# distributed-lab/era-boojum

Hardware: AMD Instinct MI355X
Metric: LDE+Merkle commit Goldilocks elems/s (2^22x256, LDE x4) (higher is better)
Workload: dtype u64 (Goldilocks); 1 GPU; C3: 2^22 rows x 256 cols, LDE x4, Poseidon2 cap 16; rows=4194304, cols=256, lde=4, cap=16, tree_hasher=poseidon2, parallelism=single, launch=stream

## Files before the change

### era-boojum_amd/csrc/bj_internal.hpp

```cpp
#pragma once
#include <hip/hip_runtime.h>
#include <stdint.h>
#include <stddef.h>
#include <stdlib.h>
#include <string.h>

namespace bj {

struct Knobs {
    bool enabled;
    uint64_t leaves_defer;
    uint64_t leaves_group;
    uint64_t inv_fold_unpaired;
    uint64_t lde_passes;
    uint64_t node_q4_max;
    uint64_t node_fused;
    uint64_t lde_own_fused;
};
inline Knobs read_knobs() {
    Knobs k{false, 0, 0, 0, 3, (uint64_t)1 << 15, 1, 1};
    const char* g = getenv("BJ_EXPERIMENTS");
    k.enabled = g && strcmp(g, "1") == 0;
    if (!k.enabled) return k;
    const char* e;
    if ((e = getenv("BJ_LEAVES_DEFER"))) k.leaves_defer = strtoull(e, nullptr, 0);
    if ((e = getenv("BJ_LEAVES_GROUP"))) k.leaves_group = strtoull(e, nullptr, 0);
    if ((e = getenv("BJ_INV_FOLD_UNPAIRED"))) k.inv_fold_unpaired = e[0] == '1';
    if ((e = getenv("BJ_LDE_PASSES"))) k.lde_passes = e[0] == '2' ? 2 : 3;
    if ((e = getenv("BJ_NODE_Q4_MAX"))) k.node_q4_max = strtoull(e, nullptr, 0);
    if ((e = getenv("BJ_NODE_FUSED"))) k.node_fused = e[0] != '0';
    if ((e = getenv("BJ_LDE_OWN_FUSED"))) k.lde_own_fused = e[0] != '0';
    return k;
}
inline const Knobs& knobs() {
    static const Knobs k = read_knobs();
    return k;
}

hipError_t launch_bitrev_scale(uint64_t* dst, size_t dst_stride, const uint64_t* src, size_t src_stride,
                               uint32_t n_cols, uint32_t log_n, uint64_t scale, hipStream_t st);
hipError_t launch_twiddles(uint64_t* out, uint32_t log_n, bool inverse, hipStream_t st);
hipError_t launch_twiddles_natural(uint64_t* out, uint32_t log_n, bool inverse, hipStream_t st);
hipError_t launch_bitrev_inplace(uint64_t* cols, size_t col_stride, uint32_t n_cols, uint32_t log_n, hipStream_t st);
hipError_t launch_power_tables(uint64_t* lo, uint64_t* hi, uint32_t log_n, uint64_t e, uint64_t scale,
                               hipStream_t st);
hipError_t launch_distribute(uint64_t* cols, size_t col_stride, uint32_t n_cols, uint32_t log_n,
                             const uint64_t* lo, const uint64_t* hi, hipStream_t st);

hipError_t launch_leaves(const uint64_t* src, size_t col_stride, uint32_t n_cols, size_t n_leaves, uint64_t* out,
                         hipStream_t st);
hipError_t launch_leaves_partial(const uint64_t* src, size_t col_stride, uint32_t n_cols, size_t n_leaves,
                                 const uint64_t* cap_in, uint64_t* out, bool final_, hipStream_t st);
hipError_t launch_leaves_chunked(const uint64_t* src, size_t col_stride, uint32_t n_cols, uint32_t log_e,
                                 size_t n_leaves, uint64_t* out, hipStream_t st);
hipError_t launch_nodes(const uint64_t* leaves, size_t n_leaves, uint32_t cap_size, uint64_t* nodes,
                        hipStream_t st);
hipError_t launch_permute(uint64_t* states, size_t count, hipStream_t st);
hipError_t launch_synthetic(uint64_t* dst, size_t col_stride, uint32_t n_cols, uint32_t log_n, uint64_t seed,
                            uint64_t col0, hipStream_t st);

hipError_t launch_gl_op(int op, const uint64_t* a, const uint64_t* b, uint64_t* out, size_t n, hipStream_t st);

hipError_t launch_twiddle_pyramid(uint64_t* out, uint32_t log_n, bool inverse, hipStream_t st);
hipError_t launch_dif(uint64_t* dst, size_t dst_stride, const uint64_t* src, size_t src_stride, uint32_t n_cols,
                      uint32_t log_n, const uint64_t* tw_pyr, bool canon_out, hipStream_t st);
hipError_t launch_lde_forward(uint64_t* lde, size_t lde_col_stride, uint32_t n_cosets, const uint64_t* raw,
                              size_t raw_stride, bool raw_bitrev, uint32_t n_cols, uint32_t log_n,
                              const uint64_t* tw_pyr, const uint64_t* pw, size_t pw_stride, hipStream_t st);

inline size_t pw_hi_len(uint32_t log_n) { return log_n > 12 ? ((size_t)1 << (log_n - 12)) : 1; }

}

namespace bj {
hipError_t launch_b2s_leaves(const uint64_t* src, size_t col_stride, uint32_t n_cols, size_t n_leaves,
                             uint64_t cols_before, const uint64_t* state_in, uint64_t* out, bool final_,
                             hipStream_t st);
hipError_t launch_b2s_leaves_chunked(const uint64_t* src, size_t col_stride, uint32_t n_cols, uint32_t log_e,
                                     size_t n_leaves, uint64_t* out, hipStream_t st);
hipError_t launch_b2s_nodes(const uint64_t* leaves, size_t n_leaves, uint32_t cap_size, uint64_t* nodes,
                            hipStream_t st);
hipError_t launch_b2s_words(const uint64_t* words, uint32_t n_words, uint64_t* out, hipStream_t st);

hipError_t launch_kc_leaves(const uint64_t* src, size_t col_stride, uint32_t n_cols, size_t n_leaves, uint64_t* out,
                            hipStream_t st);
hipError_t launch_kc_leaves_chunked(const uint64_t* src, size_t col_stride, uint32_t n_cols, uint32_t log_e,
                                    size_t n_leaves, uint64_t* out, hipStream_t st);
hipError_t launch_kc_nodes(const uint64_t* leaves, size_t n_leaves, uint32_t cap_size, uint64_t* nodes,
                           hipStream_t st);

constexpr uint32_t kMaxFold = 64;
hipError_t launch_fold(uint64_t* dst, size_t dst_stride, const uint64_t* src, size_t src_stride, uint32_t n_cols,
                       uint32_t log_m, uint32_t log_f, uint64_t s_pow_m, hipStream_t st);
hipError_t launch_fold_all(uint64_t* dst, size_t dst_col_stride, size_t dst_shard_stride, const uint64_t* src,
                           size_t src_stride, uint32_t n_cols, uint32_t log_m, uint32_t log_f, uint32_t shards,
                           const uint64_t* s_pow_m, hipStream_t st);

}

namespace bj {
bool ct_ntt_supported(uint32_t log_n);
size_t ct_table_len(uint32_t log_n);
hipError_t launch_ct_table(uint64_t* out, uint32_t log_n, bool inverse, uint64_t shift, uint64_t scale1,
                           hipStream_t st);
hipError_t launch_ct(uint64_t* dst, size_t dst_col_stride, size_t coset_stride, uint32_t n_cosets,
                     const uint64_t* src, size_t src_stride, bool src_bitrev, uint32_t n_cols, uint32_t log_n,
                     const uint64_t* tab, size_t tab_stride, uint64_t kappa, bool canon_out, hipStream_t st);
hipError_t launch_scale(uint64_t* cols, size_t stride, uint32_t n_cols, size_t n, uint64_t k, hipStream_t st);
hipError_t launch_ct_inverse_head(uint64_t* dst, size_t dst_col_stride, const uint64_t* src, size_t src_stride,
                                  uint32_t n_cols, uint32_t log_n, const uint64_t* inv_tab, hipStream_t st);

bool lde3_supported(uint32_t log_n);
size_t lde3_table_len(uint32_t log_n);
hipError_t launch_lde3_table(uint64_t* out, uint32_t log_n, uint64_t shift, hipStream_t st);
// ... 35 lines not shown
```

### era-boojum_amd/csrc/capi.hip

```cpp
#include <hip/hip_runtime.h>
#include <map>
#include <mutex>
#include <string>
#include <tuple>
#include <vector>
#include <cstring>
#include <cstdlib>
#include <cstdio>
#include <algorithm>
#include <thread>
#include <condition_variable>

#include "../../include/boojum_mi355x.h"
#include "gl.hpp"
#include "bj_internal.hpp"

namespace {

thread_local std::string g_err;

int fail(int code, const std::string& msg) {
    g_err = msg;
    return code;
}
// ... 352 lines not shown
    return BJ_OK;
}

bool inverse_fold_supported(uint32_t log_n, uint32_t log_f, uint32_t targets) {
    return use_lde3(log_n) && lde3_inv_fold_supported(log_n, log_f, targets);
}

int inverse_fold_all(const uint64_t* trace, uint32_t n_cols, size_t trace_stride, uint32_t log_n, uint32_t log_f,
                     uint32_t targets, const uint64_t* s_pow_m, uint64_t* scratch, size_t scratch_stride,
                     uint64_t* dst, size_t dst_col_stride, size_t dst_shard_stride, hipStream_t st) {
    if (!inverse_fold_supported(log_n, log_f, targets)) return fail(BJ_EINVAL, "internal: unsupported inverse fold");
    if (n_cols == 0) return BJ_OK;
    const uint64_t* inv;
    if (int r = get_ct(log_n, true, 1, &inv)) return r;
    HIP_TRY(launch_ct_inverse_head(scratch, scratch_stride, trace, trace_stride, n_cols, log_n, inv, st), "ifft");
    HIP_TRY(launch_lde3_inv_fold(dst, dst_col_stride, dst_shard_stride, scratch, scratch_stride, n_cols, log_n, log_f,
                            targets, s_pow_m, inv, st),
            "ifft fold");
    return BJ_OK;
}

uint64_t shard_shift(uint32_t log_n, uint32_t log_lde, uint32_t log_shards, uint32_t shard) {
    return ::shard_shift(log_n, log_lde, log_shards, shard);
}

static std::mutex g_pool_mu;
static std::map<int, hipMemPool_t>* g_pools = new std::map<int, hipMemPool_t>();

hipError_t pool_trim_all() {
    std::lock_guard<std::mutex> lk(g_pool_mu);
    for (auto& kv : *g_pools) {
        hipError_t e = hipMemPoolTrimTo(kv.second, 0);
        if (e != hipSuccess) return e;
    }
    return hipSuccess;
}

hipError_t pool_alloc(void** p, size_t bytes, hipStream_t st) {
    std::mutex& mu = g_pool_mu;
    std::map<int, hipMemPool_t>* pools = g_pools;
    int dev = 0;
    hipError_t e = hipGetDevice(&dev);
    if (e != hipSuccess) return e;
    hipMemPool_t pool = nullptr;
    {
        std::lock_guard<std::mutex> lk(mu);
        auto it = pools->find(dev);
        if (it == pools->end()) {
            hipMemPoolProps props;
            std::memset(&props, 0, sizeof(props));
            props.allocType = hipMemAllocationTypePinned;
            props.handleTypes = hipMemHandleTypeNone;
            props.location.type = hipMemLocationTypeDevice;
            props.location.id = dev;
            e = hipMemPoolCreate(&pool, &props);
            if (e != hipSuccess) return e;
            uint64_t keep = UINT64_MAX;
            e = hipMemPoolSetAttribute(pool, hipMemPoolAttrReleaseThreshold, &keep);
            if (e != hipSuccess) return e;
            it = pools->emplace(dev, pool).first;
        }
        pool = it->second;
    }
    return hipMallocFromPoolAsync(p, bytes ? bytes : 8, pool, st);
}
}

extern "C" {

const char* bj_last_error(void) { return g_err.c_str(); }
uint32_t bj_abi_version(void) { return (2u << 16) | 6u; }

int bj_experiment_knob(const char* name, uint64_t* value) {
    if (!name || !value) return fail(BJ_EINVAL, "bj_experiment_knob: null argument");
    const bj::Knobs& k = bj::knobs();
    if (!strcmp(name, "BJ_EXPERIMENTS")) *value = k.enabled;
    else if (!strcmp(name, "BJ_LEAVES_DEFER")) *value = k.leaves_defer;
    else if (!strcmp(name, "BJ_LEAVES_GROUP")) *value = k.leaves_group;
    else if (!strcmp(name, "BJ_INV_FOLD_UNPAIRED")) *value = k.inv_fold_unpaired;
    else if (!strcmp(name, "BJ_LDE_PASSES")) *value = k.lde_passes;
    else if (!strcmp(name, "BJ_NODE_Q4_MAX")) *value = k.node_q4_max;
    else if (!strcmp(name, "BJ_NODE_FUSED")) *value = k.node_fused;
    else if (!strcmp(name, "BJ_LDE_OWN_FUSED")) *value = k.lde_own_fused;
    else return fail(BJ_EINVAL, std::string("bj_experiment_knob: unknown knob ") + name);
    return BJ_OK;
}

int bj_release_workspace(void) {
    HIP_TRY(bj::pool_trim_all(), "hipMemPoolTrimTo");
    return BJ_OK;
}

int bj_release_tables(void) {
    Cache& c = cache();
    std::lock_guard<std::mutex> lk(c.mu);
    int cur = 0;
    HIP_TRY(hipGetDevice(&cur), "hipGetDevice");
    std::map<int, std::vector<uint64_t*>> per_dev;
    auto take = [&](auto& m, auto ptr_of) {
        for (auto& kv : m) per_dev[std::get<0>(kv.first)].push_back(ptr_of(kv.second));
        m.clear();
    };
    auto self = [](uint64_t* p) { return p; };
    take(c.tw, self);
    take(c.pyr, self);
    take(c.pw, [](const std::pair<uint64_t*, uint64_t*>& v) { return v.first; });
    take(c.lde_pw, self);
    take(c.ct, self);
    take(c.ct_lde, self);
    take(c.lde3, self);
    take(c.lde3_lde, self);
    hipError_t first = hipSuccess;
    for (auto& dv : per_dev) {
        hipError_t e = hipSetDevice(dv.first);
        if (e == hipSuccess) e = hipDeviceSynchronize();
        for (uint64_t* p : dv.second) {
            const hipError_t f = hipFree(p);
            if (e == hipSuccess) e = f;
        }
        if (first == hipSuccess) first = e;
    }
    const hipError_t e = hipSetDevice(cur);
    if (first == hipSuccess) first = e;
    if (first != hipSuccess) return hip_fail(first, "bj_release_tables");
    return BJ_OK;
}

int bj_prepare(uint32_t log_n) {
    if (int r = check_log_n(log_n)) return r;
    const uint64_t* t;
    if (int r = get_pyramid(log_n, false, &t)) return r;
    if (int r = get_pyramid(log_n, true, &t)) return r;
    if (bj::ct_ntt_supported(log_n))
        if (int r = get_ct(log_n, true, 1, &t)) return r;
    return BJ_OK;
}

int bj_precompute_twiddles_d(uint32_t log_n, int inverse, uint64_t* out_d, void* stream) {
    if (int r = check_log_n(log_n)) return r;
    if (log_n == 0) return fail(BJ_EINVAL, "twiddles need n >= 2");
    HIP_TRY(bj::launch_twiddles(out_d, log_n, inverse != 0, S(stream)), "twiddles");
    return BJ_OK;
}

int bj_precompute_twiddles_h(uint32_t log_n, int inverse, uint64_t* out_h) {
    if (int r = check_log_n(log_n)) return r;
    if (log_n == 0) return fail(BJ_EINVAL, "twiddles need n >= 2");
    const uint64_t* t;
    if (int r = get_twiddles(log_n, inverse != 0, &t)) return r;
    hipStream_t st;
    if (int r = seam_stream(&st)) return r;
    HIP_TRY(hipMemcpyAsync(out_h, t, ((size_t)1 << (log_n - 1)) * 8, hipMemcpyDeviceToHost, st), "memcpy");
    HIP_TRY(hipStreamSynchronize(st), "sync");
    return BJ_OK;
}

int bj_precompute_twiddles_natural_d(uint32_t log_n, int inverse, uint64_t* out_d, void* stream) {
    if (int r = check_log_n(log_n)) return r;
    if (log_n == 0) return fail(BJ_EINVAL, "twiddles need n >= 2");
    HIP_TRY(bj::launch_twiddles_natural(out_d, log_n, inverse != 0, S(stream)), "twiddles");
    return BJ_OK;
}

int bj_bitreverse_enumeration_d(uint64_t* cols, uint32_t n_cols, size_t col_stride, uint32_t log_n, void* stream) {
    if (int r = check_log_n(log_n)) return r;
    HIP_TRY(bj::launch_bitrev_inplace(cols, col_stride, n_cols, log_n, S(stream)), "bitreverse");
// ... 467 lines not shown
```

### era-boojum_amd/csrc/ntt_lde3.hip

```cpp
#include <hip/hip_runtime.h>
#include "gl.hpp"
#include "gl_asm.hpp"
#include "ntt_pow2.hpp"
#include "ntt_ct_common.hpp"
#include "bj_internal.hpp"

namespace bj {

namespace {

constexpr size_t L3_C = 0;
constexpr size_t L3_HA = 8192;
constexpr size_t L3_HB = L3_HA + 32;
constexpr size_t L3_F1 = L3_HB + 1024;
constexpr size_t L3_U = L3_F1 + ((size_t)1 << 18);
constexpr size_t L3_A = L3_U + 1024;
constexpr size_t L3_F2 = L3_A + ((size_t)1 << 18);

__host__ __device__ constexpr uint32_t cbrev(uint32_t x, int bits) {
    uint32_t r = 0;
    for (int i = 0; i < bits; i++) r |= ((x >> i) & 1u) << (bits - 1 - i);
    return r;
}

__device__ __forceinline__ uint32_t brev(uint32_t x, int bits) {
    return bits == 0 ? 0u : (__builtin_bitreverse32(x) >> (32 - bits));
}

__device__ __forceinline__ void prescale32_brev(uint64_t* y, const uint64_t* x, const uint64_t* f) {
#pragma unroll
    for (int k = 0; k < PT; k += 4) {
        uint32_t z0[4], z1[4];
        const uint64_t a0 = x[cbrev(k, 5)], a1 = x[cbrev(k + 1, 5)], a2 = x[cbrev(k + 2, 5)], a3 = x[cbrev(k + 3, 5)];
        glasm::mul_x4((uint32_t)a0, (uint32_t)(a0 >> 32), (uint32_t)f[k], (uint32_t)(f[k] >> 32), z0[0], z1[0],
                      (uint32_t)a1, (uint32_t)(a1 >> 32), (uint32_t)f[k + 1], (uint32_t)(f[k + 1] >> 32), z0[1], z1[1],
                      (uint32_t)a2, (uint32_t)(a2 >> 32), (uint32_t)f[k + 2], (uint32_t)(f[k + 2] >> 32), z0[2], z1[2],
                      (uint32_t)a3, (uint32_t)(a3 >> 32), (uint32_t)f[k + 3], (uint32_t)(f[k + 3] >> 32), z0[3],
                      z1[3]);
#pragma unroll
        for (int i = 0; i < 4; i++) y[k + i] = join2(z0[i], z1[i]);
    }
}

__device__ __forceinline__ __amdgpu_buffer_rsrc_t uniform_rsrc(const uint64_t* p, uint32_t bytes) {
    const uint64_t a = (uint64_t)p;
    const uint32_t lo = __builtin_amdgcn_readfirstlane((uint32_t)a);
    const uint32_t hi = __builtin_amdgcn_readfirstlane((uint32_t)(a >> 32));
    return __builtin_amdgcn_make_buffer_rsrc((void*)(((uint64_t)hi << 32) | lo), 0, (int)bytes, 0x00020000);
}

typedef unsigned int u32x2 __attribute__((ext_vector_type(2)));
__device__ __forceinline__ u32x2 as_u32x2(uint64_t v) {
    u32x2 r;
    r.x = (uint32_t)v;
    r.y = (uint32_t)(v >> 32);
    return r;
}
__device__ __forceinline__ uint64_t from_u32x2(u32x2 v) { return ((uint64_t)v.y << 32) | v.x; }

__device__ __forceinline__ void prescale32_brev_uniform(uint64_t* y, const uint64_t* x, const uint64_t* __restrict__ h) {
#pragma unroll
    for (int k8 = 0; k8 < PT; k8 += 8) {
        uint64_t hf[8];
#pragma unroll
        for (int i = 0; i < 8; i++) hf[i] = h[k8 + i];
#pragma unroll
        for (int k = k8; k < k8 + 8; k += 4) {
            uint32_t z0[4], z1[4];
            const uint64_t a0 = x[cbrev(k, 5)], a1 = x[cbrev(k + 1, 5)], a2 = x[cbrev(k + 2, 5)], a3 = x[cbrev(k + 3, 5)];
            const uint64_t f0 = hf[k - k8], f1 = hf[k - k8 + 1], f2 = hf[k - k8 + 2], f3 = hf[k - k8 + 3];
            glasm::mul_sb_x4((uint32_t)a0, (uint32_t)(a0 >> 32), (uint32_t)f0, (uint32_t)(f0 >> 32), z0[0], z1[0],
                             (uint32_t)a1, (uint32_t)(a1 >> 32), (uint32_t)f1, (uint32_t)(f1 >> 32), z0[1], z1[1],
                             (uint32_t)a2, (uint32_t)(a2 >> 32), (uint32_t)f2, (uint32_t)(f2 >> 32), z0[2], z1[2],
                             (uint32_t)a3, (uint32_t)(a3 >> 32), (uint32_t)f3, (uint32_t)(f3 >> 32), z0[3], z1[3]);
#pragma unroll
            for (int i = 0; i < 4; i++) y[k + i] = join2(z0[i], z1[i]);
        }
    }
}

__device__ __forceinline__ constexpr int c_reg(int e) { return 8 * (e / 7) + e % 7 + 1; }
template <int E0, int E1>
__device__ __forceinline__ void load_c(uint64_t* f, const uint64_t* __restrict__ c) {
#pragma unroll
    for (int e = E0; e < E1; e++) f[c_reg(e)] = c[c_reg(e)];
}

template <int E0, int E1>
__device__ __forceinline__ void prescale_c(uint64_t* y, const uint64_t* f) {
#pragma unroll
    for (int q = E0 / 4; q < E1 / 4; q++) {
        int k[4];
#pragma unroll
        for (int i = 0; i < 4; i++) k[i] = c_reg(4 * q + i);
        uint32_t z0[4], z1[4];
        glasm::mul_x4((uint32_t)y[k[0]], (uint32_t)(y[k[0]] >> 32), (uint32_t)f[k[0]], (uint32_t)(f[k[0]] >> 32), z0[0],
                      z1[0], (uint32_t)y[k[1]], (uint32_t)(y[k[1]] >> 32), (uint32_t)f[k[1]],
                      (uint32_t)(f[k[1]] >> 32), z0[1], z1[1], (uint32_t)y[k[2]], (uint32_t)(y[k[2]] >> 32),
                      (uint32_t)f[k[2]], (uint32_t)(f[k[2]] >> 32), z0[2], z1[2], (uint32_t)y[k[3]],
                      (uint32_t)(y[k[3]] >> 32), (uint32_t)f[k[3]], (uint32_t)(f[k[3]] >> 32), z0[3], z1[3]);
#pragma unroll
        for (int i = 0; i < 4; i++) y[k[i]] = join2(z0[i], z1[i]);
    }
}

__device__ __forceinline__ size_t coset_offset(uint32_t i, size_t coset_stride, size_t block_stride, uint32_t log_k) {
    return (size_t)(i >> log_k) * block_stride + (size_t)(i & ((1u << log_k) - 1)) * coset_stride;
}

template <int R>
__device__ __forceinline__ void inverse_tail13(uint64_t* x, const uint64_t* __restrict__ inv_tab, uint32_t q,
                                               uint32_t t, uint64_t* lds) {
    constexpr uint32_t LOGN = R + 13;
    const uint32_t ba = tail_base_a(t), bc = tail_base_c(t);
    const uint64_t* ext = inv_tab + ((size_t)1 << LOGN);
    uint64_t f[PT], wa[16], wb[16], wc[16];
    load32(f, ext + EXT_TA + (size_t)q * 32);
    prescale32(x, f);
    dft_p2<5, true, 0>(x);
    const uint32_t tlo = t & 7, thi = t >> 3;
    const uint32_t bb = tail_base_b(thi, tlo);
#pragma unroll
    for (int k = 0; k < PT; k++) lds[ba + tail_off_a(k)] = x[k];
    const uint64_t* tb = ext + ext_tb(R) + ((((size_t)q << 5) | thi) << 5);
// ... 224 lines not shown
#pragma unroll
                    for (uint32_t i = 0; i < OUTS; i++) {
                        h0[i] = x[2 * i];
                        h1[i] = x[2 * i + 1];
                    }
#pragma unroll
                    for (uint32_t i = 0; i < OUTS; i += 4)
                        ct_bfly_x4(h0[i], h1[i], h0[i + 1], h1[i + 1], h0[i + 2], h1[i + 2], h0[i + 3], h1[i + 3], z,
                                   z, z, z);
                } else {
                    uint64_t e[OUTS], o[OUTS];
#pragma unroll
                    for (uint32_t i = 0; i < OUTS; i++) e[i] = x[F * i];
#pragma unroll
                    for (uint32_t b = 1; b < F; b++)
                        fold_term<OUTS, F>(b < F / 2 ? e : o, x, b, zc.z[P * F + b], b == F / 2);
#pragma unroll
                    for (uint32_t i = 0; i < OUTS; i += 4)
                        for (int j = 0; j < 4; j++) {
                            h0[i + j] = e[i + j];
                            h1[i + j] = o[i + j];
                        }
#pragma unroll
                    for (uint32_t i = 0; i < OUTS; i += 4) add_sub4(h0 + i, h1 + i);
                }
#pragma unroll
                for (uint32_t i = 0; i < OUTS; i += 4) {
                    canon4(h0 + i);
                    canon4(h1 + i);
                }
                store_fold_target<OUTS>(h0, lds, P, t, dst, dst_col_stride, dst_shard_stride, c, q);
                store_fold_target<OUTS>(h1, lds, P + 1, t, dst, dst_col_stride, dst_shard_stride, c, q);
            }
            return;
        }
#pragma unroll 1
        for (uint32_t P = 0; P < shards; P++) {
            uint64_t h[OUTS];
#pragma unroll
            for (uint32_t i = 0; i < OUTS; i++) h[i] = x[F * i];
#pragma unroll
            for (uint32_t b = 1; b < F; b++) fold_term<OUTS, F>(h, x, b, zc.z[P * F + b], false);
#pragma unroll
            for (uint32_t i = 0; i < OUTS; i += 4) canon4(h + i);
            store_fold_target<OUTS>(h, lds, P, t, dst, dst_col_stride, dst_shard_stride, c, q);
        }
    }
}

template <int R>
__device__ __forceinline__ constexpr uint32_t fin_slot(uint32_t r, uint32_t o) {
    const uint32_t e = R == 5 ? (o << R) + r : r * (1u << (13 - R)) + o;
    return e + (e >> 5);
}
template <int R>
__device__ __forceinline__ constexpr uint32_t fin_p1(uint32_t t, uint32_t k) {
    constexpr int LW = 13 - R;
    return fin_slot<R>((k << (R - 5)) + cbrev(t >> LW, R - 5), t & ((1u << LW) - 1));
}
template <int R>
__device__ __forceinline__ constexpr uint32_t fin_p2(uint32_t t, uint32_t k) {
    constexpr int LW = 13 - R;
    const uint32_t h = k >> (R - 5), rl = k & ((1u << (R - 5)) - 1);
    const uint32_t p = (t >> LW) + (h << (R - 5));
    return fin_slot<R>((p << (R - 5)) + rl, t & ((1u << LW) - 1));
}
template <int R>
__device__ __forceinline__ constexpr uint32_t fin_p3(uint32_t t, uint32_t k) {
    const uint32_t P = t + 256 * k;
    return fin_slot<R>(P & ((1u << R) - 1), P >> R);
}

template <int R>
struct FinLds {
    static constexpr int LW = 13 - R, RL = R - 5;
    static constexpr uint32_t W = 1u << LW;
    static constexpr bool F1_LDS = R >= 8;
    static constexpr uint32_t F1 = F1_LDS ? 32 * W : 0;
    static constexpr uint32_t A = (1u << RL) * W;
    static constexpr uint32_t UP = (1u << RL) + 1;
    static constexpr uint32_t U = 32 * UP;
};

template <int R, int F2MODE>
__global__ __launch_bounds__(NT, 2) void lde3_final_kernel(uint64_t* lde, size_t col_stride, size_t coset_stride, size_t block_stride, uint32_t log_k,
                                                           uint32_t n_cols, uint32_t n_cosets,
                                                           const uint64_t* __restrict__ tabs, size_t tab_stride) {
    using FL = FinLds<R>;
    constexpr int LW = FL::LW, RL = FL::RL;
    constexpr uint32_t W = FL::W;
    __shared__ uint64_t lds[PAD_LDS];
    __shared__ uint64_t lf1[FL::F1 ? FL::F1 : 1];
    __shared__ uint64_t la[R > 5 && F2MODE == 1 ? FL::A : 1];
    __shared__ uint64_t lu[R > 5 && F2MODE == 1 ? FL::U : 1];
    const uint32_t t = threadIdx.x;
    const uint32_t rest = blockIdx.x >> 3;
    const uint32_t c = __builtin_amdgcn_readfirstlane(rest % n_cols);
    const uint32_t pair = ((rest / n_cols) << 3) | (blockIdx.x & 7);
    const uint32_t i = __builtin_amdgcn_readfirstlane(pair % n_cosets);
    const uint32_t T = __builtin_amdgcn_readfirstlane(pair / n_cosets);
    uint64_t* d = lde + (size_t)c * col_stride + coset_offset(i, coset_stride, block_stride, log_k) + (size_t)T * TILE;
    const uint64_t* tab = tabs + (size_t)i * tab_stride;
    const uint32_t o = t & (W - 1);
    const uint32_t M0 = T * W, M = M0 + o;
    uint64_t x[PT], y[PT], f[PT];
    const auto rd = uniform_rsrc(d, 8u * TILE);
    constexpr uint32_t NF1 = FL::F1_LDS ? FL::F1 / NT : 1;
    uint64_t f1v[NF1];
    if constexpr (FL::F1_LDS) {
#pragma unroll
        for (uint32_t j = 0; j < NF1; j++) {
            const uint32_t e = t + j * NT;
            f1v[j] = tab[L3_F1 + ((size_t)(e >> LW) << 13) + M0 + (e & (W - 1))];
        }
    }
#pragma unroll
    for (int k = 0; k < PT; k++) x[k] = from_u32x2(__builtin_amdgcn_raw_buffer_load_b64(rd, (int)(t * 8), k * 2048, 0));
    if constexpr (R > 5 && F2MODE == 1) {
        la[t] = tab[L3_A + ((size_t)(t >> LW) << 13) + M0 + (t & (W - 1))];
#pragma unroll
        for (uint32_t e = t; e < (32u << RL); e += NT) lu[(e >> RL) * FL::UP + (e & ((1u << RL) - 1))] = tab[L3_U + e];
    }
    uint64_t g2[F2MODE == 0 && R > 5 ? PT : 1];
    if constexpr (F2MODE == 0 && R > 5) {
        const auto rf = uniform_rsrc(tab + L3_F2 + M0, 8u << (R + 13));
        const int vf = (int)((o + ((t >> LW) << 13)) * 8);
#pragma unroll
        for (int k = 0; k < PT; k++) {
            const uint32_t h = k >> RL, rl = k & ((1u << RL) - 1);
            g2[k] = from_u32x2(__builtin_amdgcn_raw_buffer_load_b64(rf, vf, (int)((rl * 32 + (h << RL)) << 16), 0));
        }
    }
    if constexpr (FL::F1_LDS) {
#pragma unroll
        for (uint32_t j = 0; j < NF1; j++) lf1[t + j * NT] = f1v[j];
        __syncthreads();
#pragma unroll
        for (int k = 0; k < PT; k++) f[k] = lf1[k * W + o];
    } else {
        const uint64_t* f1 = tab + L3_F1 + M;
#pragma unroll
        for (int k = 0; k < PT; k++) f[k] = f1[(size_t)k << 13];
    }
    prescale32_brev(y, x, f);
    dft_p2<5, false, 0>(y);
    const uint32_t b1 = fin_p1<R>(t, 0);
#pragma unroll
    for (int k = 0; k < PT; k++) lds[b1 + (fin_p1<R>(0, k) - fin_p1<R>(0, 0))] = y[k];
    if constexpr (R > 5) {
        const uint32_t pl = t >> LW;
        if constexpr (F2MODE == 1) {
            if constexpr (!FL::F1_LDS) __syncthreads();
            uint64_t a[PT];
#pragma unroll
            for (int k = 0; k < PT; k++) {
                const uint32_t h = k >> RL, rl = k & ((1u << RL) - 1);
                a[k] = la[rl * W + o];
                f[k] = lu[(pl + (h << RL)) * FL::UP + rl];
            }
            prescale32(f, a);
        } else {
#pragma unroll
            for (int k = 0; k < PT; k++) f[k] = g2[k];
        }
        __syncthreads();
        const uint32_t b2 = fin_p2<R>(t, 0);
#pragma unroll
        for (int k = 0; k < PT; k++) y[k] = lds[b2 + (fin_p2<R>(0, k) - fin_p2<R>(0, 0))];
        prescale32(y, f);
        dft_p2_groups<RL, false>(y);
#pragma unroll
        for (int k = 0; k < PT; k++) lds[b2 + (fin_p2<R>(0, k) - fin_p2<R>(0, 0))] = y[k];
    }
    __syncthreads();
    const uint32_t b3 = fin_p3<R>(t, 0);
#pragma unroll
    for (int k = 0; k < PT; k++) y[k] = lds[b3 + (fin_p3<R>(0, k) - fin_p3<R>(0, 0))];
#pragma unroll
    for (int k = 0; k < PT; k += 4) canon4(y + k);
#pragma unroll
    for (int k = 0; k < PT; k++) __builtin_amdgcn_raw_buffer_store_b64(as_u32x2(y[k]), rd, (int)(t * 8), k * 2048, 0);
}

__global__ void lde3_table_kernel(uint64_t* out, uint32_t log_n, uint64_t w_n, uint64_t s, size_t len) {
    const size_t n = (size_t)1 << log_n;
    const uint32_t R = log_n - 13;
    for (size_t idx = blockIdx.x * (size_t)blockDim.x + threadIdx.x; idx < len;
         idx += (size_t)gridDim.x * blockDim.x) {
        uint64_t v;
        if (idx < L3_HA) {
            const uint32_t G = (uint32_t)idx >> 3, j = (uint32_t)idx & 7;
            const uint64_t sigma = gl::mul(s, gl::pow(w_n, gl::bitrev32(G, 10)));
            v = gl::pow(sigma, (n >> 13) * j);
        } else if (idx < L3_HB) {
            v = gl::pow(s, (n >> 5) * (idx - L3_HA));
        } else if (idx < L3_F1) {
            const uint32_t j = (uint32_t)(idx - L3_HB);
            const uint64_t sigma = gl::mul(s, gl::pow(w_n, gl::bitrev32(j >> 5, 5)));
            v = gl::pow(sigma, (n >> 10) * (j & 31));
        } else if (idx < L3_U) {
            const uint32_t j = (uint32_t)(idx - L3_F1);
            const uint32_t M = j & 8191, k = j >> 13;
            const uint64_t sigma = gl::mul(s, gl::pow(w_n, gl::bitrev32(M, 13)));
            v = gl::pow(sigma, (uint64_t)k << (R - 5));
        } else if (idx < L3_A) {
            const uint32_t j = (uint32_t)(idx - L3_U);
            const uint32_t p = j >> (R - 5), rl = j & ((1u << (R - 5)) - 1);
            v = (j >> R) ? 0 : gl::pow(gl::pow(w_n, 8192), (uint64_t)gl::bitrev32(p, 5) * rl);
        } else if (idx < L3_F2) {
            const uint32_t j = (uint32_t)(idx - L3_A);
            const uint32_t M = j & 8191, rl = j >> 13;
            const uint64_t sigma = gl::mul(s, gl::pow(w_n, gl::bitrev32(M, 13)));
            v = (rl >> (R - 5)) ? 0 : gl::pow(sigma, rl);
        } else {
            const size_t j = idx - L3_F2;
            const uint32_t M = (uint32_t)(j & 8191), rest = (uint32_t)(j >> 13);
            const uint32_t p = rest & 31, rl = rest >> 5;
            const uint64_t sigma = gl::mul(s, gl::pow(w_n, gl::bitrev32(M * 32 + p, 18)));
            v = gl::pow(sigma, rl);
        }
        out[idx] = gl::canon(v);
    }
}

template <int R>
void launch_lde3_R(uint64_t* lde, size_t col_stride, size_t coset_stride, size_t block_stride, uint32_t log_k, uint32_t n_cosets, const uint64_t* src,
                   size_t src_stride, uint64_t* mono, size_t mono_stride, uint32_t n_cols, const uint64_t* inv_tab,
                   const uint64_t* tabs, size_t tab_stride, hipStream_t st, uint32_t passes) {
    const dim3 gm(n_cols << R);
    if (!(passes & LDE3_MID))
        ;
    else if (inv_tab && mono)
        hipLaunchKernelGGL((lde3_mid_kernel<R, true, true>), gm, dim3(NT), 0, st, src, src_stride, mono, mono_stride,
                           lde, col_stride, coset_stride, block_stride, log_k, n_cols, n_cosets, inv_tab, tabs, tab_stride);
    else if (inv_tab)
        hipLaunchKernelGGL((lde3_mid_kernel<R, true, false>), gm, dim3(NT), 0, st, src, src_stride, mono,
                           mono_stride, lde, col_stride, coset_stride, block_stride, log_k, n_cols, n_cosets, inv_tab, tabs, tab_stride);
    else
        hipLaunchKernelGGL((lde3_mid_kernel<R, false, false>), gm, dim3(NT), 0, st, src, src_stride, mono,
                           mono_stride, lde, col_stride, coset_stride, block_stride, log_k, n_cols, n_cosets, inv_tab, tabs, tab_stride);
    const dim3 gf((n_cols * n_cosets) << R);
    if (passes & LDE3_FINAL)
        hipLaunchKernelGGL((lde3_final_kernel<R, 0>), gf, dim3(NT), 0, st, lde, col_stride, coset_stride, block_stride,
                           log_k, n_cols, n_cosets, tabs, tab_stride);
}

}

bool lde3_supported(uint32_t log_n) { return log_n >= 18 && log_n <= 23; }

size_t lde3_table_len(uint32_t log_n) {
    return log_n > 18 ? L3_F2 + ((size_t)1 << log_n) : L3_F2;
}

hipError_t launch_lde3_table(uint64_t* out, uint32_t log_n, uint64_t shift, hipStream_t st) {
    if (!lde3_supported(log_n)) return hipErrorInvalidValue;
    const size_t len = lde3_table_len(log_n);
    size_t blocks = (len + 255) / 256;
    if (blocks > 16384) blocks = 16384;
    hipLaunchKernelGGL(lde3_table_kernel, dim3((unsigned)blocks), dim3(256), 0, st, out, log_n,
                       gl::domain_generator(log_n), gl::canon(shift), len);
    return hipGetLastError();
}

hipError_t launch_lde3(uint64_t* lde, size_t col_stride, size_t coset_stride, uint32_t n_cosets, const uint64_t* src,
                       size_t src_stride, uint64_t* mono, size_t mono_stride, uint32_t n_cols, uint32_t log_n,
                       const uint64_t* inv_tab, const uint64_t* tabs, size_t tab_stride, hipStream_t st,
                       uint32_t log_k, size_t block_stride, uint32_t passes) {
    if (n_cols == 0 || n_cosets == 0) return hipSuccess;
    if (log_k > 31) log_k = 31;
    if (!lde3_supported(log_n)) return hipErrorInvalidValue;
    if (((uint64_t)n_cols * n_cosets) << (log_n - 13) > (0xffffffffull / NT)) return hipErrorInvalidValue;
#define BJ_LDE3(RR)                                                                                              \
    launch_lde3_R<RR>(lde, col_stride, coset_stride, block_stride, log_k, n_cosets, src, src_stride, mono, mono_stride, n_cols, inv_tab, \
                      tabs, tab_stride, st, passes)
    switch (log_n - 13) {
        case 5: BJ_LDE3(5); break;
        case 6: BJ_LDE3(6); break;
        case 7: BJ_LDE3(7); break;
        case 8: BJ_LDE3(8); break;
        case 9: BJ_LDE3(9); break;
        default: BJ_LDE3(10); break;
    }
#undef BJ_LDE3
    return hipGetLastError();
}

namespace {
template <int R>
void launch_lde3_inv_fold_R(uint64_t* dst, size_t dst_col_stride, size_t dst_shard_stride, const uint64_t* src,
                            size_t src_stride, uint32_t n_cols, uint32_t log_f, uint32_t shards, uint32_t paired,
                            const uint64_t* inv_tab, const InvFoldZ& zc, hipStream_t st) {
    const dim3 g(n_cols << R);
#define BJ_INV(LF)                                                                                             \
    hipLaunchKernelGGL((lde3_inv_fold_kernel<R, LF>), g, dim3(NT), 0, st, src, src_stride, dst, dst_col_stride, \
                       dst_shard_stride, n_cols, shards, paired, inv_tab, zc)
    switch (log_f) {
        case 1: BJ_INV(1); break;
        case 2: BJ_INV(2); break;
        default: BJ_INV(3); break;
    }
#undef BJ_INV
}
}

bool lde3_inv_fold_supported(uint32_t log_n, uint32_t log_f, uint32_t shards) {
    return lde3_supported(log_n) && log_f >= 1 && log_f <= 3 && shards >= 1 &&
           (size_t)shards << log_f <= kInvFoldConsts;
}

hipError_t launch_lde3_inv_fold(uint64_t* dst, size_t dst_col_stride, size_t dst_shard_stride, const uint64_t* src,
                                size_t src_stride, uint32_t n_cols, uint32_t log_n, uint32_t log_f, uint32_t shards,
                                const uint64_t* s_pow_m, const uint64_t* inv_tab, hipStream_t st) {
    if (n_cols == 0) return hipSuccess;
    if (!lde3_inv_fold_supported(log_n, log_f, shards)) return hipErrorInvalidValue;
    if (((uint64_t)n_cols << (log_n - 13)) > 0xffffffffull / NT) return hipErrorInvalidValue;
    InvFoldZ zc{};
    const uint32_t F = 1u << log_f;
    for (uint32_t P = 0; P < shards; P++) {
        uint64_t acc = 1;
        for (uint32_t a = 0; a < F; a++) {
            zc.z[P * F + gl::bitrev32(a, log_f)] = acc;
            acc = gl::mul(acc, s_pow_m[P]);
        }
    }
    uint32_t paired = shards % 2 == 0 && !knobs().inv_fold_unpaired;
    for (uint32_t P = 0; paired && P < shards; P += 2)
        paired = gl::canon(s_pow_m[P + 1]) == gl::canon(gl::sub(0, s_pow_m[P]));
#define BJ_INVR(RR) \
    launch_lde3_inv_fold_R<RR>(dst, dst_col_stride, dst_shard_stride, src, src_stride, n_cols, log_f, shards, paired, \
                               inv_tab, zc, st)
    switch (log_n - 13) {
        case 5: BJ_INVR(5); break;
        case 6: BJ_INVR(6); break;
        case 7: BJ_INVR(7); break;
        case 8: BJ_INVR(8); break;
        case 9: BJ_INVR(9); break;
        default: BJ_INVR(10); break;
    }
#undef BJ_INVR
    return hipGetLastError();
}

}
```

Baseline: 5.832 billion elems/s.

## Process multiple columns per block in LDE final kernel with prefetch of next column

Result: no change. 5.827 billion elems/s (-0.1%).

```diff
diff --git a/era-boojum_amd/csrc/bj_internal.hpp b/era-boojum_amd/csrc/bj_internal.hpp
--- a/era-boojum_amd/csrc/bj_internal.hpp
+++ b/era-boojum_amd/csrc/bj_internal.hpp
@@ -16,9 +16,10 @@
     uint64_t node_q4_max;
     uint64_t node_fused;
     uint64_t lde_own_fused;
+    uint64_t lde_final_cols;
 };
 inline Knobs read_knobs() {
-    Knobs k{false, 0, 0, 0, 3, (uint64_t)1 << 15, 1, 1};
+    Knobs k{false, 0, 0, 0, 3, (uint64_t)1 << 15, 1, 1, 0};
     const char* g = getenv("BJ_EXPERIMENTS");
     k.enabled = g && strcmp(g, "1") == 0;
     if (!k.enabled) return k;
@@ -30,6 +31,7 @@
     if ((e = getenv("BJ_NODE_Q4_MAX"))) k.node_q4_max = strtoull(e, nullptr, 0);
     if ((e = getenv("BJ_NODE_FUSED"))) k.node_fused = e[0] != '0';
     if ((e = getenv("BJ_LDE_OWN_FUSED"))) k.lde_own_fused = e[0] != '0';
+    if ((e = getenv("BJ_LDE_FINAL_COLS"))) k.lde_final_cols = strtoull(e, nullptr, 0);
     return k;
 }
 inline const Knobs& knobs() {
diff --git a/era-boojum_amd/csrc/capi.hip b/era-boojum_amd/csrc/capi.hip
--- a/era-boojum_amd/csrc/capi.hip
+++ b/era-boojum_amd/csrc/capi.hip
@@ -458,6 +458,7 @@
     else if (!strcmp(name, "BJ_NODE_Q4_MAX")) *value = k.node_q4_max;
     else if (!strcmp(name, "BJ_NODE_FUSED")) *value = k.node_fused;
     else if (!strcmp(name, "BJ_LDE_OWN_FUSED")) *value = k.lde_own_fused;
+    else if (!strcmp(name, "BJ_LDE_FINAL_COLS")) *value = k.lde_final_cols;
     else return fail(BJ_EINVAL, std::string("bj_experiment_knob: unknown knob ") + name);
     return BJ_OK;
 }
diff --git a/era-boojum_amd/csrc/ntt_lde3.hip b/era-boojum_amd/csrc/ntt_lde3.hip
--- a/era-boojum_amd/csrc/ntt_lde3.hip
+++ b/era-boojum_amd/csrc/ntt_lde3.hip
@@ -27,9 +27,10 @@
     return bits == 0 ? 0u : (__builtin_bitreverse32(x) >> (32 - bits));
 }
 
-__device__ __forceinline__ void prescale32_brev(uint64_t* y, const uint64_t* x, const uint64_t* f) {
-#pragma unroll
-    for (int k = 0; k < PT; k += 4) {
+template <int K0, int K1>
+__device__ __forceinline__ void prescale_brev(uint64_t* y, const uint64_t* x, const uint64_t* f) {
+#pragma unroll
+    for (int k = K0; k < K1; k += 4) {
         uint32_t z0[4], z1[4];
         const uint64_t a0 = x[cbrev(k, 5)], a1 = x[cbrev(k + 1, 5)], a2 = x[cbrev(k + 2, 5)], a3 = x[cbrev(k + 3, 5)];
         glasm::mul_x4((uint32_t)a0, (uint32_t)(a0 >> 32), (uint32_t)f[k], (uint32_t)(f[k] >> 32), z0[0], z1[0],
@@ -40,6 +41,9 @@
 #pragma unroll
         for (int i = 0; i < 4; i++) y[k + i] = join2(z0[i], z1[i]);
     }
+}
+__device__ __forceinline__ void prescale32_brev(uint64_t* y, const uint64_t* x, const uint64_t* f) {
+    prescale_brev<0, PT>(y, x, f);
 }
 
 __device__ __forceinline__ __amdgpu_buffer_rsrc_t uniform_rsrc(const uint64_t* p, uint32_t bytes) {
@@ -430,7 +434,13 @@
     static constexpr uint32_t U = 32 * UP;
 };
 
-template <int R, int F2MODE>
+constexpr int kFinalCols = 4;
+inline int final_cols() {
+    const uint64_t k = knobs().lde_final_cols;
+    return k == 1 || k == 2 || k == 4 || k == 8 ? (int)k : kFinalCols;
+}
+
+template <int R, int F2MODE, int K = 1>
 __global__ __launch_bounds__(NT, 2) void lde3_final_kernel(uint64_t* lde, size_t col_stride, size_t coset_stride, size_t block_stride, uint32_t log_k,
                                                            uint32_t n_cols, uint32_t n_cosets,
                                                            const uint64_t* __restrict__ tabs, size_t tab_stride) {
@@ -442,17 +452,18 @@
     __shared__ uint64_t la[R > 5 && F2MODE == 1 ? FL::A : 1];
     __shared__ uint64_t lu[R > 5 && F2MODE == 1 ? FL::U : 1];
     const uint32_t t = threadIdx.x;
+    const uint32_t nb = (n_cols + K - 1) / K;
     const uint32_t rest = blockIdx.x >> 3;
-    const uint32_t c = __builtin_amdgcn_readfirstlane(rest % n_cols);
-    const uint32_t pair = ((rest / n_cols) << 3) | (blockIdx.x & 7);
+    const uint32_t c0 = __builtin_amdgcn_readfirstlane((rest % nb) * K);
+    const uint32_t pair = ((rest / nb) << 3) | (blockIdx.x & 7);
     const uint32_t i = __builtin_amdgcn_readfirstlane(pair % n_cosets);
     const uint32_t T = __builtin_amdgcn_readfirstlane(pair / n_cosets);
-    uint64_t* d = lde + (size_t)c * col_stride + coset_offset(i, coset_stride, block_stride, log_k) + (size_t)T * TILE;
+    const uint32_t kc = K == 1 ? 1u : __builtin_amdgcn_readfirstlane(min((uint32_t)K, n_cols - c0));
+    uint64_t* d = lde + (size_t)c0 * col_stride + coset_offset(i, coset_stride, block_stride, log_k) + (size_t)T * TILE;
     const uint64_t* tab = tabs + (size_t)i * tab_stride;
     const uint32_t o = t & (W - 1);
     const uint32_t M0 = T * W, M = M0 + o;
     uint64_t x[PT], y[PT], f[PT];
-    const auto rd = uniform_rsrc(d, 8u * TILE);
     constexpr uint32_t NF1 = FL::F1_LDS ? FL::F1 / NT : 1;
     uint64_t f1v[NF1];
     if constexpr (FL::F1_LDS) {
@@ -462,8 +473,12 @@
             f1v[j] = tab[L3_F1 + ((size_t)(e >> LW) << 13) + M0 + (e & (W - 1))];
         }
     }
-#pragma unroll
-    for (int k = 0; k < PT; k++) x[k] = from_u32x2(__builtin_amdgcn_raw_buffer_load_b64(rd, (int)(t * 8), k * 2048, 0));
+    {
+        const auto rd = uniform_rsrc(d, 8u * TILE);
+#pragma unroll
+        for (int k = 0; k < PT; k++)
+            x[k] = from_u32x2(__builtin_amdgcn_raw_buffer_load_b64(rd, (int)(t * 8), k * 2048, 0));
+    }
     if constexpr (R > 5 && F2MODE == 1) {
         la[t] = tab[L3_A + ((size_t)(t >> LW) << 13) + M0 + (t & (W - 1))];
 #pragma unroll
@@ -483,51 +498,78 @@
 #pragma unroll
         for (uint32_t j = 0; j < NF1; j++) lf1[t + j * NT] = f1v[j];
         __syncthreads();
-#pragma unroll
-        for (int k = 0; k < PT; k++) f[k] = lf1[k * W + o];
-    } else {
-        const uint64_t* f1 = tab + L3_F1 + M;
-#pragma unroll
-        for (int k = 0; k < PT; k++) f[k] = f1[(size_t)k << 13];
-    }
-    prescale32_brev(y, x, f);
-    dft_p2<5, false, 0>(y);
-    const uint32_t b1 = fin_p1<R>(t, 0);
-#pragma unroll
-    for (int k = 0; k < PT; k++) lds[b1 + (fin_p1<R>(0, k) - fin_p1<R>(0, 0))] = y[k];
-    if constexpr (R > 5) {
-        const uint32_t pl = t >> LW;
-        if constexpr (F2MODE == 1) {
-            if constexpr (!FL::F1_LDS) __syncthreads();
-            uint64_t a[PT];
-#pragma unroll
-            for (int k = 0; k < PT; k++) {
-                const uint32_t h = k >> RL, rl = k & ((1u << RL) - 1);
-                a[k] = la[rl * W + o];
-                f[k] = lu[(pl + (h << RL)) * FL::UP + rl];
+    }
+    const uint32_t b1 = fin_p1<R>(t, 0), b3 = fin_p3<R>(t, 0);
+#pragma unroll 1
+    for (uint32_t j = 0; j < kc; j++, d += col_stride) {
+        if constexpr (K == 1) {
+            if constexpr (FL::F1_LDS) {
+#pragma unroll
+                for (int k = 0; k < PT; k++) f[k] = lf1[k * W + o];
+            } else {
+                const uint64_t* f1 = tab + L3_F1 + M;
+#pragma unroll
+                for (int k = 0; k < PT; k++) f[k] = f1[(size_t)k << 13];
             }
-            prescale32(f, a);
+            prescale32_brev(y, x, f);
         } else {
-#pragma unroll
-            for (int k = 0; k < PT; k++) f[k] = g2[k];
-        }
-        __syncthreads();
-        const uint32_t b2 = fin_p2<R>(t, 0);
-#pragma unroll
-        for (int k = 0; k < PT; k++) y[k] = lds[b2 + (fin_p2<R>(0, k) - fin_p2<R>(0, 0))];
-        prescale32(y, f);
-        dft_p2_groups<RL, false>(y);
-#pragma unroll
-        for (int k = 0; k < PT; k++) lds[b2 + (fin_p2<R>(0, k) - fin_p2<R>(0, 0))] = y[k];
-    }
-    __syncthreads();
-    const uint32_t b3 = fin_p3<R>(t, 0);
-#pragma unroll
-    for (int k = 0; k < PT; k++) y[k] = lds[b3 + (fin_p3<R>(0, k) - fin_p3<R>(0, 0))];
-#pragma unroll
-    for (int k = 0; k < PT; k += 4) canon4(y + k);
-#pragma unroll
-    for (int k = 0; k < PT; k++) __builtin_amdgcn_raw_buffer_store_b64(as_u32x2(y[k]), rd, (int)(t * 8), k * 2048, 0);
+            const auto r1 = uniform_rsrc(tab + L3_F1 + M0, 8u << 18);
+#pragma unroll
+            for (int k = 0; k < PT / 2; k++)
+                f[k] = FL::F1_LDS ? lf1[k * W + o]
+                                  : from_u32x2(__builtin_amdgcn_raw_buffer_load_b64(r1, (int)(o * 8), k << 16, 0));
+            prescale_brev<0, PT / 2>(y, x, f);
+#pragma unroll
+            for (int k = PT / 2; k < PT; k++)
+                f[k] = FL::F1_LDS ? lf1[k * W + o]
+                                  : from_u32x2(__builtin_amdgcn_raw_buffer_load_b64(r1, (int)(o * 8), k << 16, 0));
+            prescale_brev<PT / 2, PT>(y, x, f);
+        }
+        dft_p2<5, false, 0>(y);
+        if constexpr (K > 1) __syncthreads();
+#pragma unroll
+        for (int k = 0; k < PT; k++) lds[b1 + (fin_p1<R>(0, k) - fin_p1<R>(0, 0))] = y[k];
+        if constexpr (R > 5) {
+            const uint32_t pl = t >> LW;
+            if constexpr (F2MODE == 1) {
+                if constexpr (!FL::F1_LDS) __syncthreads();
+                uint64_t a[PT];
+#pragma unroll
+                for (int k = 0; k < PT; k++) {
+                    const uint32_t h = k >> RL, rl = k & ((1u << RL) - 1);
+                    a[k] = la[rl * W + o];
+                    f[k] = lu[(pl + (h << RL)) * FL::UP + rl];
+                }
+                prescale32(f, a);
+            } else {
+#pragma unroll
+                for (int k = 0; k < PT; k++) f[k] = g2[k];
+            }
+            __syncthreads();
+            const uint32_t b2 = fin_p2<R>(t, 0);
+#pragma unroll
+            for (int k = 0; k < PT; k++) y[k] = lds[b2 + (fin_p2<R>(0, k) - fin_p2<R>(0, 0))];
+            prescale32(y, f);
+            dft_p2_groups<RL, false>(y);
+#pragma unroll
+            for (int k = 0; k < PT; k++) lds[b2 + (fin_p2<R>(0, k) - fin_p2<R>(0, 0))] = y[k];
+        }
+        __syncthreads();
+        if constexpr (K > 1) {
+            const bool more = j + 1 < kc;
+            const auto rn = uniform_rsrc(more ? d + col_stride : d, more ? 8u * TILE : 0u);
+#pragma unroll
+            for (int k = 0; k < PT; k++)
+                x[k] = from_u32x2(__builtin_amdgcn_raw_buffer_load_b64(rn, (int)(t * 8), k * 2048, 0));
+        }
+        const auto rd = uniform_rsrc(d, 8u * TILE);
+#pragma unroll
+        for (int k = 0; k < PT; k++) y[k] = lds[b3 + (fin_p3<R>(0, k) - fin_p3<R>(0, 0))];
+#pragma unroll
+        for (int k = 0; k < PT; k += 4) canon4(y + k);
+#pragma unroll
+        for (int k = 0; k < PT; k++) __builtin_amdgcn_raw_buffer_store_b64(as_u32x2(y[k]), rd, (int)(t * 8), k * 2048, 0);
+    }
 }
 
 __global__ void lde3_table_kernel(uint64_t* out, uint32_t log_n, uint64_t w_n, uint64_t s, size_t len) {
@@ -587,10 +629,17 @@
     else
         hipLaunchKernelGGL((lde3_mid_kernel<R, false, false>), gm, dim3(NT), 0, st, src, src_stride, mono,
                            mono_stride, lde, col_stride, coset_stride, block_stride, log_k, n_cols, n_cosets, inv_tab, tabs, tab_stride);
-    const dim3 gf((n_cols * n_cosets) << R);
-    if (passes & LDE3_FINAL)
-        hipLaunchKernelGGL((lde3_final_kernel<R, 0>), gf, dim3(NT), 0, st, lde, col_stride, coset_stride, block_stride,
-                           log_k, n_cols, n_cosets, tabs, tab_stride);
+    if (!(passes & LDE3_FINAL)) return;
+#define BJ_FINAL(KK)                                                                                               \
+    hipLaunchKernelGGL((lde3_final_kernel<R, 0, KK>), dim3((((n_cols + KK - 1) / KK) * n_cosets) << R), dim3(NT), 0, st, \
+                       lde, col_stride, coset_stride, block_stride, log_k, n_cols, n_cosets, tabs, tab_stride)
+    switch (final_cols()) {
+        case 1: BJ_FINAL(1); break;
+        case 2: BJ_FINAL(2); break;
+        case 4: BJ_FINAL(4); break;
+        default: BJ_FINAL(8); break;
+    }
+#undef BJ_FINAL
 }
 
 }
@@ -618,7 +667,8 @@
     if (n_cols == 0 || n_cosets == 0) return hipSuccess;
     if (log_k > 31) log_k = 31;
     if (!lde3_supported(log_n)) return hipErrorInvalidValue;
-    if (((uint64_t)n_cols * n_cosets) << (log_n - 13) > (0xffffffffull / NT)) return hipErrorInvalidValue;
+    const uint64_t runs = ((uint64_t)n_cols + final_cols() - 1) / final_cols();
+    if (std::max<uint64_t>(n_cols, runs * n_cosets) << (log_n - 13) > (0xffffffffull / NT)) return hipErrorInvalidValue;
 #define BJ_LDE3(RR)                                                                                              \
     launch_lde3_R<RR>(lde, col_stride, coset_stride, block_stride, log_k, n_cosets, src, src_stride, mono, mono_stride, n_cols, inv_tab, \
                       tabs, tab_stride, st, passes)
```
